# bottledspace/refraction-raytracing-dxr

Measured on AMD Instinct MI355X. Metric: Mrays/s (primary+refracted) at 1920x1080, monkey.obj, higher is better.
Workload: dtype f32

## Files before the change

refraction_raytracing_dxr_amd/csrc/rr_device.h:

```cpp
#pragma once
#include <hip/hip_runtime.h>
#include "rr_types.h"

namespace rr {

struct f3 { float x, y, z; };

__device__ __forceinline__ f3 mk3(float x, float y, float z) { f3 r; r.x = x; r.y = y; r.z = z; return r; }
__device__ __forceinline__ f3 sub3(f3 a, f3 b) { return mk3(a.x - b.x, a.y - b.y, a.z - b.z); }
__device__ __forceinline__ f3 neg3(f3 a) { return mk3(-a.x, -a.y, -a.z); }
__device__ __forceinline__ f3 scale3(f3 a, float s) { return mk3(a.x * s, a.y * s, a.z * s); }
__device__ __forceinline__ float dot3(f3 a, f3 b) { return fmaf(a.z, b.z, fmaf(a.y, b.y, a.x * b.x)); }
__device__ __forceinline__ f3 cross3(f3 a, f3 b)
{
    return mk3(fmaf(a.y, b.z, -(a.z * b.y)), fmaf(a.z, b.x, -(a.x * b.z)), fmaf(a.x, b.y, -(a.y * b.x)));
}
__device__ __forceinline__ f3 normalize3(f3 a)
{
    float inv = 1.0f / sqrtf(dot3(a, a));
    return scale3(a, inv);
}

__device__ __forceinline__ float rr_atan2f(float y, float x)
{
    const float q = fabsf(y) / fabsf(x);
    const bool big = q > 2.414213562373095f, mid = !big && q > 0.4142135623730950f;
    const float num = big ? -1.0f : mid ? q - 1.0f : q;
    const float den = big ? q : mid ? q + 1.0f : 1.0f;
    const float y0 = big ? 1.5707963267948966f : mid ? 0.7853981633974483f : 0.0f;
    const float xr = num / den;
    const float z = xr * xr;
    const float p = ((8.05374449538e-2f * z - 1.38776856032e-1f) * z + 1.99777106478e-1f) * z - 3.33329491539e-1f;
    const float r = p * z * xr + xr;
    float a = y0 + r;
    if (x < 0.0f) a = 3.14159265358979323846f - a;
    float res = y < 0.0f ? -a : a;
    if (x == 0.0f) res = y > 0.0f ? 1.5707963267948966f : -1.5707963267948966f;
    if (y == 0.0f) res = (x > 0.0f || (x == 0.0f && !__builtin_signbit(x))) ? y
                                                                             : (__builtin_signbit(y) ? -3.14159265358979323846f : 3.14159265358979323846f);
    if (x != x || y != y) res = __builtin_nanf("");
    return res;
}

__device__ __forceinline__ float rr_acosf(float x)
{
    const float ax = fabsf(x);
    const bool outer = ax > 0.5f;
    const float a = outer ? sqrtf(0.5f * (1.0f - ax)) : ax;
    const float z = a * a;
    const float p = ((((4.2163199048e-2f * z + 2.4181311049e-2f) * z + 4.5470025998e-2f) * z + 7.4953002686e-2f) * z
                     + 1.6666752422e-1f);
    const float r = p * z * a + a;
    const float two_r = 2.0f * r;
    float res = outer ? (x < 0.0f ? 3.14159265358979323846f - two_r : two_r) : 1.5707963267948966f - (x < 0.0f ? -r : r);
    if (!(x >= -1.0f && x <= 1.0f)) res = __builtin_nanf("");
    return res;
}

__device__ __forceinline__ uint32_t ftou(float f)
{
    uint32_t r;
    asm("v_cvt_u32_f32 %0, %1" : "=v"(r) : "v"(f));
    return r;
}

__device__ __forceinline__ uint32_t unorm8(float x)
{
    float c;
    asm("v_max_f32 %0, %1, 0" : "=v"(c) : "v"(x));
    asm("v_min_f32 %0, %1, 1.0" : "=v"(c) : "v"(c));
    return ftou(c * 255.0f + 0.5f);
}

struct HitRec {
    float t, U, V, ad;
    uint32_t prim;
    uint32_t leaf;
    uint32_t inst;
    bool hit;
};

struct TravCounters { uint32_t nodes, tris, node_trips = 0, leaf_trips = 0; };
__device__ __forceinline__ bool first_active_lane()
{
    return (int)(threadIdx.x & 63u) == __ffsll((long long)__ballot(1)) - 1;
}

constexpr uint32_t CULL_BACK = 0x10u, CULL_FRONT = 0x20u;
constexpr uint32_t RAY_FLAG_ACCEPT_FIRST_HIT = 0x4u;

struct BoxRay {
    f3 inv;
    f3 kn, kf;
    bool sx, sy, sz;
};
__device__ __forceinline__ void box_axis(float o, float d, float eps_w, float org, float cell, float& inv_g, float& kn, float& kf, bool& neg)
{
    const float dg = fabsf(d) < 1e-20f ? copysignf(1e-20f, d) : d;
    const float inv = __builtin_amdgcn_rcpf(dg);
    const float oi = (org - o) * inv;
    const float pad = fmaf(fabsf(oi), 1e-6f, fabsf(inv) * eps_w);
    kn = oi - pad;
    kf = oi + pad;
    inv_g = inv * cell;
    neg = inv < 0.0f;
}
__device__ __forceinline__ BoxRay box_ray(f3 O, f3 D, float scene_scale, const QGrid& g)
{
    const float eps_w = 1e-5f * fmaxf(fmaxf(fabsf(O.x), fabsf(O.y)), fmaxf(fabsf(O.z), scene_scale));
    BoxRay r;
    box_axis(O.x, D.x, eps_w, g.org[0], g.cell[0], r.inv.x, r.kn.x, r.kf.x, r.sx);
    box_axis(O.y, D.y, eps_w, g.org[1], g.cell[1], r.inv.y, r.kn.y, r.kf.y, r.sy);
    box_axis(O.z, D.z, eps_w, g.org[2], g.cell[2], r.inv.z, r.kn.z, r.kf.z, r.sz);
    return r;
}

struct NodeQ { uint4 a, b; };
__device__ __forceinline__ NodeQ load_node(const QNode* __restrict__ nodes, int node)
{
    const uint4* q = reinterpret_cast<const uint4*>(reinterpret_cast<const char*>(nodes) + (uint32_t)node);
    NodeQ n;
    n.a = q[0]; n.b = q[1];
    return n;
}
struct GlobalNodes {
    __device__ __forceinline__ NodeQ load(const QNode* __restrict__ nodes, int node) const { return load_node(nodes, node); }
};
struct LdsNodes {
    const char* base;
    __device__ __forceinline__ NodeQ load(const QNode* __restrict__, int node) const
    {
        const uint4* q = reinterpret_cast<const uint4*>(base + (uint32_t)node);
        NodeQ n;
        n.a = q[0]; n.b = q[1];
        return n;
    }
};


constexpr int TRAV_DONE = (int)0x80000000;

typedef float v2f __attribute__((ext_vector_type(2)));
__device__ __forceinline__ v2f splat2(float x) { v2f r = { x, x }; return r; }
__device__ __forceinline__ v2f mk2(float x, float y) { v2f r = { x, y }; return r; }

__device__ __forceinline__ float vmax3(float a, float b, float c) { float r; asm("v_max3_f32 %0, %1, %2, %3" : "=v"(r) : "v"(a), "v"(b), "v"(c)); return r; }
__device__ __forceinline__ float vmin3(float a, float b, float c) { float r; asm("v_min3_f32 %0, %1, %2, %3" : "=v"(r) : "v"(a), "v"(b), "v"(c)); return r; }
__device__ __forceinline__ float vmax2(float a, float b) { float r; asm("v_max_f32 %0, %1, %2" : "=v"(r) : "v"(a), "v"(b)); return r; }
__device__ __forceinline__ float vmin2(float a, float b) { float r; asm("v_min_f32 %0, %1, %2" : "=v"(r) : "v"(a), "v"(b)); return r; }

typedef _Float16 h2v __attribute__((ext_vector_type(2)));
__device__ __forceinline__ h2v as_h2(uint32_t w) { return __builtin_bit_cast(h2v, w); }
#define RR_PLANE2(word, inv, k) mk2(fmaf((float)as_h2(word).x, inv, k), fmaf((float)as_h2(word).y, inv, k))
__device__ __forceinline__ void box2_hit(const BoxRay& r, const NodeQ& n, float tmin, float tmax,
                                         bool& h0, bool& h1, float& tn0, float& tn1)
{
    const uint32_t lox = n.a.x, loy = n.a.y, loz = n.a.z, hix = n.a.w, hiy = n.b.x, hiz = n.b.y;
    const v2f nx = RR_PLANE2(r.sx ? hix : lox, r.inv.x, r.kn.x);
    const v2f ny = RR_PLANE2(r.sy ? hiy : loy, r.inv.y, r.kn.y);
    const v2f nz = RR_PLANE2(r.sz ? hiz : loz, r.inv.z, r.kn.z);
    const v2f fx = RR_PLANE2(r.sx ? lox : hix, r.inv.x, r.kf.x);
    const v2f fy = RR_PLANE2(r.sy ? loy : hiy, r.inv.y, r.kf.y);
    const v2f fz = RR_PLANE2(r.sz ? loz : hiz, r.inv.z, r.kf.z);
    tn0 = vmax2(vmax3(nx.x, ny.x, nz.x), tmin);
    tn1 = vmax2(vmax3(nx.y, ny.y, nz.y), tmin);
    const float tf0 = vmin2(vmin3(fx.x, fy.x, fz.x), tmax);
    const float tf1 = vmin2(vmin3(fx.y, fy.y, fz.y), tmax);
    h0 = tn0 <= tf0;
    h1 = tn1 <= tf1;
}

constexpr int STACK_STRIDE = 64;
template <class E> struct StackCodec;
template <> struct StackCodec<uint32_t> {
    static __device__ __forceinline__ uint32_t enc(int ref) { return (uint32_t)ref; }
    static __device__ __forceinline__ int dec(uint32_t v) { return (int)v; }
};
template <> struct StackCodec<uint16_t> {
    static __device__ __forceinline__ uint16_t enc(int ref) { const int n = ref >> 5; return (uint16_t)(n < ref ? n : ref); }
    static __device__ __forceinline__ int dec(uint16_t v) { const int s = (int)(int16_t)v, n = s << 5; return n > s ? n : s; }
};

template <class E>
__device__ __forceinline__ int node_step(const BoxRay& br, const NodeQ& n, float tmin, float tmax, E*& top, const E* floor)
{
    bool h0, h1;
    float tn0, tn1;
    box2_hit(br, n, tmin, tmax, h0, h1, tn0, tn1);
    const int c0 = (int)n.b.z, c1 = (int)n.b.w;
    const bool both = h0 && h1, swap = tn1 < tn0;
    const int nearc = (h0 && !(h1 && swap)) ? c0 : c1;
    int next = (h0 || h1) ? nearc : TRAV_DONE;
    if (both) { *top = StackCodec<E>::enc(swap ? c0 : c1); top += STACK_STRIDE; }
    if (!(h0 || h1) && top > floor) { top -= STACK_STRIDE; next = StackCodec<E>::dec(*top); }
    return next;
}

struct Diag { uint32_t* trips; uint32_t stride = 4; };
__device__ __forceinline__ void diag_trip(const Diag& d, int which = 0)
{
    if (d.trips) { const unsigned long long m = __ballot(1); if ((int)(threadIdx.x & 63u) == __ffsll((long long)m) - 1) d.trips[which * d.stride] += 1u; }
}


__device__ __forceinline__ bool tri_accept(const TriRec* __restrict__ tris, uint32_t leaf, f3 O, f3 D, float tmin, uint32_t cull,
                                           float& t, uint32_t& prim)
{
    const float4* q = reinterpret_cast<const float4*>(tris + leaf);
    float4 a = q[0], b = q[1], c = q[2];
    f3 v0 = mk3(a.x, a.y, a.z), e1 = mk3(b.x, b.y, b.z), e2 = mk3(c.x, c.y, c.z);
    prim = __float_as_uint(a.w);
    f3 pv = cross3(D, e2);
    float det = dot3(e1, pv);
    if (cull & CULL_BACK) { if (!(det > 0.0f)) return false; }
    else if (cull & CULL_FRONT) { if (!(det < 0.0f)) return false; }
    else if (!(det != 0.0f)) return false;
    f3 tv = sub3(O, v0);
    float U = dot3(tv, pv);
    f3 qv = cross3(tv, e1);
    float V = dot3(D, qv);
    float T = dot3(e2, qv);
    float ad = det;
    if (det < 0.0f) { U = -U; V = -V; T = -T; ad = -det; }
    if (U < 0.0f || V < 0.0f || U + V > ad) return false;
    t = T / ad;
    return t > tmin;
}

__device__ __forceinline__ void tri_test(const TriRec* __restrict__ tris, uint32_t leaf, f3 O, f3 D, float tmin,
                                         uint32_t cull, uint32_t inst, HitRec& best)
{
    float t;
    uint32_t prim;
    if (!tri_accept(tris, leaf, O, D, tmin, cull, t, prim)) return;
    if (t < best.t || (t == best.t && best.hit && (inst < best.inst || (inst == best.inst && prim < tris[best.leaf].prim)))) {
        best.t = t; best.leaf = leaf; best.inst = inst;
        best.hit = true;
    }
}

__device__ __forceinline__ float hit_attributes(const TriRec* __restrict__ tris, f3 O, f3 D, HitRec& best)
{
    const float4* q = reinterpret_cast<const float4*>(tris + best.leaf);
    float4 a = q[0], b = q[1], c = q[2];
    f3 v0 = mk3(a.x, a.y, a.z), e1 = mk3(b.x, b.y, b.z), e2 = mk3(c.x, c.y, c.z);
    f3 pv = cross3(D, e2);
    float det = dot3(e1, pv);
    f3 tv = sub3(O, v0);
    float U = dot3(tv, pv);
    f3 qv = cross3(tv, e1);
    float V = dot3(D, qv);
    float ad = det;
    if (det < 0.0f) { U = -U; V = -V; ad = -det; }
    best.U = U; best.V = V; best.ad = ad; best.prim = __float_as_uint(a.w);
    return det;
}

__device__ __forceinline__ void hits_begin(HitRec& best, float tmax)
{
    best.t = tmax; best.hit = false; best.prim = 0; best.leaf = 0; best.inst = 0; best.U = 0.0f; best.V = 0.0f;
    best.ad = 1.0f;
}
__device__ __forceinline__ float hit_bound(const HitRec& best) { return best.t; }
__device__ __forceinline__ bool hit_found(const HitRec& best) { return best.hit; }
__device__ __forceinline__ void leaf_test(const TriRec* __restrict__ tris, uint32_t leaf, f3 O, f3 D, float tmin, uint32_t cull,
                                          uint32_t inst, HitRec& best)
{
    tri_test(tris, leaf, O, D, tmin, cull, inst, best);
}
__device__ __forceinline__ void hits_end_blas(const TriRec* __restrict__ tris, f3 O, f3 D, HitRec& best)
{
    if (best.hit) hit_attributes(tris, O, D, best);
}

template <int KB, bool COUNT>
struct MultiHits {
    float t[KB];
    uint32_t leaf[KB], inst[KB];
    float tmax;
    uint32_t count;
};
template <int KB, bool COUNT>
__device__ __forceinline__ void hits_begin(MultiHits<KB, COUNT>& m, float tmax)
{
#pragma unroll
    for (int j = 0; j < KB; ++j) { m.t[j] = tmax; m.leaf[j] = 0; m.inst[j] = 0; }
    m.tmax = tmax; m.count = 0;
}
template <int KB, bool COUNT>
__device__ __forceinline__ float hit_bound(const MultiHits<KB, COUNT>& m) { return COUNT ? m.tmax : m.t[KB - 1]; }
template <int KB, bool COUNT>
__device__ __forceinline__ bool hit_found(const MultiHits<KB, COUNT>&) { return false; }
template <int KB, bool COUNT>
__device__ __forceinline__ void leaf_test(const TriRec* __restrict__ tris, uint32_t leaf, f3 O, f3 D, float tmin, uint32_t cull,
                                          uint32_t inst, MultiHits<KB, COUNT>& m)
{
    float t;
    uint32_t prim;
    if (!tri_accept(tris, leaf, O, D, tmin, cull, t, prim) || !(t < m.tmax)) return;
    if (COUNT) m.count++;
    bool before[KB];
#pragma unroll
    for (int j = 0; j < KB; ++j)
        before[j] = t < m.t[j] || (t == m.t[j] && (inst < m.inst[j] || (inst == m.inst[j] && prim < tris[m.leaf[j]].prim)));
    if (!before[KB - 1]) return;
#pragma unroll
    for (int j = KB - 1; j > 0; --j) {
        if (before[j - 1]) { m.t[j] = m.t[j - 1]; m.leaf[j] = m.leaf[j - 1]; m.inst[j] = m.inst[j - 1]; }
        else if (before[j]) { m.t[j] = t; m.leaf[j] = leaf; m.inst[j] = inst; }
    }
    if (before[0]) { m.t[0] = t; m.leaf[0] = leaf; m.inst[0] = inst; }
}
template <int KB, bool COUNT>
__device__ __forceinline__ void hits_end_blas(const TriRec* __restrict__, f3, f3, MultiHits<KB, COUNT>&) {}

__device__ __forceinline__ bool leaf_phase_due(int n_in)
{
    const int quarter = n_in >> 2;
    const int thr = quarter > 2 ? quarter : 2;
    return __popcll(__ballot(1)) + thr <= n_in;
}

template <bool STATS, class E, class NS = GlobalNodes, bool ANY = false, class H = HitRec>
__device__ __forceinline__ void walk_blas(const QNode* __restrict__ nodes, const TriRec* __restrict__ tris, int root, const BoxRay& br,
                                          f3 O, f3 D, float tmin, uint32_t cull, uint32_t inst, H& best, E* stk,
                                          TravCounters& cnt, const Diag dg = Diag{ nullptr }, const NS ns = NS{},
                                          bool any_lane = false)
{
    E* top = stk;
    int node = root;
    for (;;) {
        const int n_in = __popcll(__ballot(node >= 0));
        while (node >= 0) {
            if (leaf_phase_due(n_in)) break;
            diag_trip(dg);
            const NodeQ q = ns.load(nodes, node);
            if (STATS) { cnt.nodes++; if (first_active_lane()) cnt.node_trips++; }
            node = node_step(br, q, tmin, hit_bound(best), top, stk);
        }
        if (node < 0 && node != TRAV_DONE) {
            diag_trip(dg, 1);
            if (STATS) { cnt.tris++; if (first_active_lane()) cnt.leaf_trips++; }
            leaf_test(tris, (uint32_t)~node, O, D, tmin, cull, inst, best);
            if (ANY && any_lane && hit_found(best)) { top = stk; node = TRAV_DONE; }
            else if (top > stk) { top -= STACK_STRIDE; node = StackCodec<E>::dec(*top); } else node = TRAV_DONE;
        }
        if (__ballot(node != TRAV_DONE) == 0ull) break;
    }
}

template <bool STATS, class E, class NS = GlobalNodes, class H = HitRec>
__device__ __forceinline__ void trace_blas(const BlasDev& bl, f3 O, f3 D, float tmin, uint32_t cull, uint32_t inst,
                                           H& best, E* stk, TravCounters& cnt, const Diag dg = Diag{ nullptr },
                                           const NS ns = NS{})
{
    const BoxRay br = box_ray(O, D, bl.scale, bl.grid);
    walk_blas<STATS, E, NS>(bl.nodes, bl.tris, 0, br, O, D, tmin, cull, inst, best, stk, cnt, dg, ns);
    hits_end_blas(bl.tris, O, D, best);
}

template <int G> __device__ __forceinline__ uint32_t grp_next(uint32_t v);
template <int G> __device__ __forceinline__ uint32_t grp_prev(uint32_t v);
template <> __device__ __forceinline__ uint32_t grp_next<4>(uint32_t v) { return (uint32_t)__builtin_amdgcn_update_dpp(0, (int)v, 0x39, 0xf, 0xf, true); }
template <> __device__ __forceinline__ uint32_t grp_prev<4>(uint32_t v) { return (uint32_t)__builtin_amdgcn_update_dpp(0, (int)v, 0x93, 0xf, 0xf, true); }
template <> __device__ __forceinline__ uint32_t grp_next<2>(uint32_t v) { return (uint32_t)__builtin_amdgcn_update_dpp(0, (int)v, 0xb1, 0xf, 0xf, true); }
template <> __device__ __forceinline__ uint32_t grp_prev<2>(uint32_t v) { return grp_next<2>(v); }
template <int G> __device__ __forceinline__ float grp_min_f(float v)
{
    float m = fminf(v, __uint_as_float((uint32_t)__builtin_amdgcn_update_dpp(0, (int)__float_as_uint(v), 0xb1, 0xf, 0xf, true)));
    if (G == 4) m = fminf(m, __uint_as_float((uint32_t)__builtin_amdgcn_update_dpp(0, (int)__float_as_uint(m), 0x4e, 0xf, 0xf, true)));
    return m;
}
template <int G> __device__ __forceinline__ uint32_t grp_min_u(uint32_t v)
{
    uint32_t o = (uint32_t)__builtin_amdgcn_update_dpp(0, (int)v, 0xb1, 0xf, 0xf, true);
    uint32_t m = v < o ? v : o;
    if (G == 4) { o = (uint32_t)__builtin_amdgcn_update_dpp(0, (int)m, 0x4e, 0xf, 0xf, true); m = m < o ? m : o; }
    return m;
}

template <int G, bool STATS, class E>
__device__ __forceinline__ void trace_blas_group(const BlasDev& bl, bool alive, unsigned long long m_alive, f3 O, f3 D, float tmin, float tmax,
                                                 uint32_t cull, HitRec& best, E* stk, uint32_t* ww, uint32_t lane, TravCounters& cnt)
{
    const uint32_t rank = __builtin_amdgcn_mbcnt_hi((uint32_t)(m_alive >> 32), __builtin_amdgcn_mbcnt_lo((uint32_t)m_alive, 0u));
    const uint32_t n_rays = (uint32_t)__popcll(m_alive);
    if (alive) {
        ww[0 * 64 + rank] = __float_as_uint(O.x); ww[1 * 64 + rank] = __float_as_uint(O.y); ww[2 * 64 + rank] = __float_as_uint(O.z);
        ww[3 * 64 + rank] = __float_as_uint(D.x); ww[4 * 64 + rank] = __float_as_uint(D.y); ww[5 * 64 + rank] = __float_as_uint(D.z);
        ww[6 * 64 + rank] = __float_as_uint(tmax); ww[7 * 64 + rank] = cull; ww[8 * 64 + rank] = __float_as_uint(tmin);
    }
    const uint32_t g = lane / G;
    const bool work = g < n_rays;
    const uint32_t gs = work ? g : 0u;
    const f3 Og = mk3(__uint_as_float(ww[0 * 64 + gs]), __uint_as_float(ww[1 * 64 + gs]), __uint_as_float(ww[2 * 64 + gs]));
    const f3 Dg = mk3(__uint_as_float(ww[3 * 64 + gs]), __uint_as_float(ww[4 * 64 + gs]), __uint_as_float(ww[5 * 64 + gs]));
    const float tmaxg = __uint_as_float(ww[6 * 64 + gs]);
    const uint32_t cullg = ww[7 * 64 + gs];
    const float tming = __uint_as_float(ww[8 * 64 + gs]);
    asm volatile("s_waitcnt lgkmcnt(0)" ::: "memory");

    const BoxRay br = box_ray(Og, Dg, bl.scale, bl.grid);
    const QNode* __restrict__ nodes = bl.nodes;
    E* const col0 = stk - lane;
    E* top = stk;
    E* bot = stk;
    int node = (work && (lane % G) == 0u) ? 0 : TRAV_DONE;
    HitRec b;
    b.t = tmaxg; b.hit = false; b.prim = 0; b.leaf = 0; b.inst = 0; b.U = 0.0f; b.V = 0.0f; b.ad = 1.0f;
    float tq = tmaxg;
    for (;;) {
        const int n_in = __popcll(__ballot(node >= 0));
        while (node >= 0) {
            if (leaf_phase_due(n_in)) break;
            const NodeQ q = load_node(nodes, node);
            if (STATS) { cnt.nodes++; if (first_active_lane()) cnt.node_trips++; }
            node = node_step(br, q, tming, tq, top, bot);
        }
        if (node < 0 && node != TRAV_DONE) {
            if (STATS) { cnt.tris++; if (first_active_lane()) cnt.leaf_trips++; }
            tri_test(bl.tris, (uint32_t)~node, Og, Dg, tming, cullg, 0u, b);
            if (top > bot) { top -= STACK_STRIDE; node = StackCodec<E>::dec(*top); } else node = TRAV_DONE;
        }
        tq = grp_min_f<G>(b.t);
        const bool idle = node == TRAV_DONE;
        const uint32_t nb_bot = grp_next<G>((uint32_t)(bot - col0)), nb_has = grp_next<G>(top > bot ? 1u : 0u);
        const uint32_t thief_idle = grp_prev<G>(idle ? 1u : 0u);
        if (idle && nb_has) node = StackCodec<E>::dec(col0[nb_bot]);
        if (top > bot && thief_idle) bot += STACK_STRIDE;
        if (__ballot(node != TRAV_DONE) == 0ull) break;
    }
    const float tw = grp_min_f<G>(b.hit ? b.t : 3.0e38f);
    const bool cand = b.hit && b.t == tw;
    const uint32_t prim = cand ? bl.tris[b.leaf].prim : 0xffffffffu;
    const uint32_t pw = grp_min_u<G>(prim);
    const uint32_t lw = ~grp_min_u<G>((cand && prim == pw) ? ~b.leaf : 0xffffffffu);
    if (work && (lane % G) == 0u) { ww[0 * 64 + g] = __float_as_uint(tw); ww[1 * 64 + g] = tw < 3.0e38f ? lw : 0xffffffffu; }
    best.t = tmax; best.hit = false; best.prim = 0; best.leaf = 0; best.inst = 0; best.U = 0.0f; best.V = 0.0f; best.ad = 1.0f;
    if (alive) {
        const uint32_t l = ww[1 * 64 + rank];
        if (l != 0xffffffffu) { best.t = __uint_as_float(ww[0 * 64 + rank]); best.leaf = l; best.hit = true; }
    }
    asm volatile("s_waitcnt lgkmcnt(0)" ::: "memory");
    if (best.hit) hit_attributes(bl.tris, O, D, best);
}

__device__ __forceinline__ f3 xform_point(const float* m, f3 p)
{
    return mk3(((m[0] * p.x + m[1] * p.y) + m[2] * p.z) + m[3],
               ((m[4] * p.x + m[5] * p.y) + m[6] * p.z) + m[7],
               ((m[8] * p.x + m[9] * p.y) + m[10] * p.z) + m[11]);
}
__device__ __forceinline__ f3 xform_dir(const float* m, f3 p)
{
    return mk3((m[0] * p.x + m[1] * p.y) + m[2] * p.z,
               (m[4] * p.x + m[5] * p.y) + m[6] * p.z,
               (m[8] * p.x + m[9] * p.y) + m[10] * p.z);
}

__device__ __forceinline__ InstDev inst_record(const InstDev* __restrict__ insts, uint32_t ii)
{
    const uint32_t iu = (uint32_t)__builtin_amdgcn_readfirstlane((int)ii);
    InstDev r;
    if (__ballot(ii != iu) == 0ull) r = insts[iu];
    else r = insts[ii];
    return r;
}

__device__ __forceinline__ void ray_in_instance(const InstDev& in, f3 O, f3 D, f3& Oc, f3& Dc)
{
    Oc = O; Dc = D;
    if (!in.identity) { Oc = xform_point(in.inv, O); Dc = xform_dir(in.inv, D); }
}
__device__ __forceinline__ void hits_end_scene(const SceneDev& sc, f3 O, f3 D, HitRec& best)
{
    if (best.hit) {
        const InstDev in = inst_record(sc.insts, best.inst);
        f3 Oh = O, Dh = D;
        if (!in.identity) { Oh = xform_point(in.inv, O); Dh = xform_dir(in.inv, D); }
        hit_attributes(sc.pool_tris, Oh, Dh, best);
    }
}
template <int KB, bool COUNT>
__device__ __forceinline__ void hits_end_scene(const SceneDev&, f3, f3, MultiHits<KB, COUNT>&) {}

struct HitRecFace : HitRec { bool front; };
__device__ __forceinline__ void hits_end_blas(const TriRec* __restrict__ tris, f3 O, f3 D, HitRecFace& best)
{
    best.front = false;
    if (best.hit) best.front = hit_attributes(tris, O, D, best) > 0.0f;
}
__device__ __forceinline__ void hits_end_scene(const SceneDev& sc, f3 O, f3 D, HitRecFace& best)
{
    best.front = false;
    if (best.hit) {
        const InstDev in = inst_record(sc.insts, best.inst);
        f3 Oh = O, Dh = D;
        if (!in.identity) { Oh = xform_point(in.inv, O); Dh = xform_dir(in.inv, D); }
        const float det = hit_attributes(sc.pool_tris, Oh, Dh, best);
        best.front = (det > 0.0f) != ((in.flags & 0x2u) != 0u);
    }
}

template <bool STATS, bool TLAS, class E = uint32_t, class NS = GlobalNodes, bool QUERY = false, class H = HitRec>
__device__ __forceinline__ void trace_scene(const SceneDev& sc, f3 O, f3 D, float tmin, float tmax, uint32_t flags,
                                            H& best, E* stk_e, TravCounters& cnt,
                                            const Diag dg = Diag{ nullptr }, const NS ns = NS{},
                                            uint32_t ray_mask = 0xffu, bool any_lane = false)
{
    hits_begin(best, tmax);
    if (!TLAS && QUERY) {
        const BoxRay br = box_ray(O, D, sc.blas0.scale, sc.blas0.grid);
        walk_blas<STATS, E, NS, true>(sc.blas0.nodes, sc.blas0.tris, (ray_mask & 0xffu) ? 0 : TRAV_DONE, br, O, D, tmin, flags, 0u,
                                      best, stk_e, cnt, dg, ns, any_lane);
        hits_end_blas(sc.blas0.tris, O, D, best);
        return;
    }
    if (!TLAS) {
        trace_blas<STATS, E, NS>(sc.blas0, O, D, tmin, flags, 0u, best, stk_e, cnt, dg, ns);
        return;
    }
    E* stk = stk_e;
    const QNode* __restrict__ nodes = sc.pool_nodes;
    E* top = stk;
    int node = 0;
    const BoxRay br = box_ray(O, D, sc.scale, sc.grid);
    for (;;) {
        while (node >= 0) {
            const NodeQ q = load_node(nodes, node);
            if (STATS) { cnt.nodes++; if (first_active_lane()) cnt.node_trips++; }
            node = node_step(br, q, tmin, hit_bound(best), top, stk);
        }
        if (node == TRAV_DONE) break;
        if (STATS && first_active_lane()) cnt.leaf_trips++;
        const uint32_t ii = (uint32_t)~node - sc.n_pool_tris;
        const InstDev in = inst_record(sc.insts, ii);
        if (in.mask & (QUERY ? ray_mask : 0xffu)) {
            uint32_t f = flags;
            if (in.flags & 0x1u) f &= ~(CULL_BACK | CULL_FRONT);
            else if (in.flags & 0x2u) {
                if (f & CULL_BACK) f = (f & ~CULL_BACK) | CULL_FRONT;
                else if (f & CULL_FRONT) f = (f & ~CULL_FRONT) | CULL_BACK;
            }
            f3 Oc = O, Dc = D;
            if (!in.identity) { Oc = xform_point(in.inv, O); Dc = xform_dir(in.inv, D); }
            const BoxRay bi = box_ray(Oc, Dc, in.scale, in.grid);
            walk_blas<STATS, E, GlobalNodes, QUERY>(nodes, sc.pool_tris, (int)in.root, bi, Oc, Dc, tmin, f, ii, best, top, cnt,
                                                    Diag{ nullptr }, GlobalNodes{}, any_lane);
        }
        if (QUERY && any_lane && hit_found(best)) node = TRAV_DONE;
        else if (top > stk) { top -= STACK_STRIDE; node = StackCodec<E>::dec(*top); } else node = TRAV_DONE;
    }
    hits_end_scene(sc, O, D, best);
}

__device__ __forceinline__ f3 env_lookup(const SceneDev& sc, f3 r)
{
    if (!sc.env) return mk3(0.0f, 0.0f, 0.0f);
    float at = rr_atan2f(r.x, r.z);
    float ac = rr_acosf(r.y);
    float theta = (float)sc.env_w * (at / 3.14159f + 1.0f) / 2;
    float phi = (float)sc.env_h * (ac / 3.14159f);
    uint32_t ix = ftou(theta), iy = ftou(phi);
    if (ix >= (uint32_t)sc.env_w || iy >= (uint32_t)sc.env_h) return mk3(0.0f, 0.0f, 0.0f);
    float4 t = sc.env[(size_t)iy * (uint32_t)sc.env_w + ix];
    return mk3(t.x, t.y, t.z);
}

__device__ __forceinline__ f3 reflect_ray(f3 I, f3 N)
{
    float k = 2.0f * dot3(N, I);
    return mk3(I.x - k * N.x, I.y - k * N.y, I.z - k * N.z);
}

__device__ __forceinline__ bool refract_ray(f3& R, f3 I, f3 N, float eta)
{
    float c = dot3(N, I);
    float k = 1.0f - (eta * eta) * (1.0f - c * c);
    if (k < 0.0f) return false;
    float a = eta * c + sqrtf(k);
    R = normalize3(mk3(eta * I.x - a * N.x, eta * I.y - a * N.y, eta * I.z - a * N.z));
    return true;
}

__device__ __forceinline__ f3 camera_ray_dir(const float* M, float sx, float sy)
{
    f3 R;
    R.x = (sx * M[0] + sy * M[1]) + M[3];
    R.y = (sx * M[4] + sy * M[5]) + M[7];
    R.z = (sx * M[8] + sy * M[9]) + M[11];
    return normalize3(R);
}

template <bool TLAS>
__device__ __forceinline__ f3 shading_normal(const SceneDev& sc, const HitRec& h)
{
    const float4* q = reinterpret_cast<const float4*>((!TLAS ? sc.blas0.nrms : sc.pool_nrms) + h.leaf);
    float4 a = q[0], b = q[1], c = q[2];
    float u = h.U / h.ad, v = h.V / h.ad;
    f3 A = mk3(a.x, a.y, a.z);
    f3 BA = sub3(mk3(b.x, b.y, b.z), A), CA = sub3(mk3(c.x, c.y, c.z), A);
    f3 Nr = mk3(fmaf(v, CA.x, fmaf(u, BA.x, A.x)), fmaf(v, CA.y, fmaf(u, BA.y, A.y)), fmaf(v, CA.z, fmaf(u, BA.z, A.z)));
    const InstDev in = TLAS ? inst_record(sc.insts, h.inst) : InstDev{};
    if (TLAS && !in.identity) {
        const float* w = in.inv;
        Nr = mk3((w[0] * Nr.x + w[4] * Nr.y) + w[8] * Nr.z,
                 (w[1] * Nr.x + w[5] * Nr.y) + w[9] * Nr.z,
                 (w[2] * Nr.x + w[6] * Nr.y) + w[10] * Nr.z);
    }
    return normalize3(Nr);
}

__device__ __forceinline__ uint32_t wave_reduce_add(uint32_t v)
{
    uint32_t t;
    t = v + __builtin_amdgcn_update_dpp(0u, v, 0x111, 0xf, 0xf, true);
    t = t + __builtin_amdgcn_update_dpp(0u, v, 0x112, 0xf, 0xf, true);
    t = t + __builtin_amdgcn_update_dpp(0u, v, 0x113, 0xf, 0xf, true);
    t = t + __builtin_amdgcn_update_dpp(0u, t, 0x114, 0xf, 0xe, true);
    t = t + __builtin_amdgcn_update_dpp(0u, t, 0x118, 0xf, 0xc, true);
    t = t + __builtin_amdgcn_update_dpp(0u, t, 0x142, 0xa, 0xf, true);
    t = t + __builtin_amdgcn_update_dpp(0u, t, 0x143, 0xc, 0xf, true);
    return (uint32_t)__builtin_amdgcn_readlane((int)t, 63);
}

}
```

refraction_raytracing_dxr_amd/csrc/rr_render_lds.hip:

```cpp
#include <hip/hip_runtime.h>
#include "rr_render_common.h"

namespace rr {

__device__ __forceinline__ BlockPos lds_tile_block(const DispatchDev& a, const LdsDispatch& q, uint32_t u, uint32_t j)
{
    BlockPos p;
    const uint32_t tile = a.n_frames == 1u ? u : __umulhi(u, q.div_frames);
    p.frame = u - tile * a.n_frames;
    p.tile_local = tile;
    p.tile_ok = tile < a.n_local_tiles;
    p.bg = false;
    const uint32_t ty = a.tiles_x == 1u ? tile : __umulhi(tile, q.div_tiles_x), tx = tile - ty * a.tiles_x;
    p.px0 = (j & 3u) * 8u; p.py0 = (j >> 2) * 8u;
    p.x0 = tx * TILE + p.px0; p.y0 = ty * TILE + p.py0;
    return p;
}

__device__ __forceinline__ BlockPos lds_rect_block(const DispatchDev& a, const LdsDispatch& q, uint32_t u, uint32_t j)
{
    BlockPos p;
    const uint32_t strip = a.n_frames == 1u ? u : __umulhi(u, q.div_frames), per_row = q.rect_bw >> 2;
    p.frame = u - strip * a.n_frames;
    const uint32_t row = per_row == 1u ? strip : __umulhi(strip, q.div_per_row), col = strip - row * per_row;
    p.tile_local = 0u; p.tile_ok = true; p.bg = false;
    p.px0 = 0u; p.py0 = 0u;
    p.x0 = q.rx0 + col * 32u + j * 8u; p.y0 = q.ry0 + row * 8u;
    return p;
}

template <int NW, int WGS, bool STATS, bool DIAG = false>
__global__ __launch_bounds__(NW * 64, NW * WGS / 4) void k_render_lds(SceneDev sc, DispatchDev a, LdsDispatch q)
{
    typedef uint16_t E;
    __shared__ uint32_t diag_tr[3 * 16];
    __shared__ uint32_t wg_arrived;
    __shared__ unsigned long long wg_share[16];
    if (threadIdx.x == 0) wg_arrived = 0u;
    if (threadIdx.x < 16) wg_share[threadIdx.x] = 0ull;
    const unsigned long long diag_t0 = DIAG ? __builtin_amdgcn_s_memtime() : 0ull;
    unsigned long long diag_wait = 0ull, diag_render = 0ull, diag_n = 0ull;
    unsigned long long diag_worst = 0ull, diag_worst_trips = 0ull;
    if (DIAG && threadIdx.x < 48) diag_tr[threadIdx.x] = 0;
    extern __shared__ __attribute__((aligned(16))) uint32_t lds[];
    {
        const uint4* __restrict__ src = reinterpret_cast<const uint4*>(sc.blas0.nodes);
        uint4* dst = reinterpret_cast<uint4*>(lds);
        for (uint32_t i = threadIdx.x; i < q.node_bytes / 16u; i += NW * 64) dst[i] = src[i];
    }
    __syncthreads();
    const unsigned long long diag_t1 = DIAG ? __builtin_amdgcn_s_memtime() : 0ull;
    const uint32_t wave = __builtin_amdgcn_readfirstlane(threadIdx.x >> 6), lane = threadIdx.x & 63u;
    const LdsNodes ns{ reinterpret_cast<const char*>(lds) };
    MemPark park{ q.park + (size_t)(blockIdx.x * NW + wave) * ((size_t)q.park_slots * 8 * 64) + lane };
    E* stk = reinterpret_cast<E*>(reinterpret_cast<char*>(lds) + q.node_bytes) + wave * (q.stack_entries * 64u) + lane;
    const uint32_t lx = compact1by1(lane), ly = compact1by1(lane >> 1);

    LaneStats st;
    stats_clock_begin<STATS>(st);
    auto in_rect = [&](const BlockPos& bp) { return bp.x0 >= q.rx0 && bp.x0 < q.rx1 && bp.y0 >= q.ry0 && bp.y0 < q.ry1; };
    const uint32_t NQ = q.n_queues;
    uint32_t home = (blockIdx.x * NW + wave) % NQ;
    if (q.home_xcc) { uint32_t xcc; asm volatile("s_getreg_b32 %0, hwreg(HW_REG_XCC_ID)" : "=s"(xcc)); home = (xcc & 7u) % NQ; }
    uint32_t phase = 0, qi = home, tried = 0;
    for (;;) {
        BlockPos bp;
        bool have = false;
        while (!have) {
            {
                uint32_t got = 0xffffffffu, got_u = 0u;
                for (;;) {
                    const unsigned long long mine = lane < (uint32_t)NW ? wg_share[lane] : 0ull;
                    const uint32_t mh = (uint32_t)(mine >> 32);
                    const unsigned long long m = __ballot(mh != 0u && (uint32_t)mine < ((mh & 0x80000000u) ? 16u : 4u));
                    if (m == 0ull) break;
                    const unsigned long long from_own = m >> wave << wave;
                    const uint32_t sl = (uint32_t)__ffsll((long long)(from_own ? from_own : m)) - 1u;
                    unsigned long long v = 0ull;
                    if (lane == 0) v = atomicAdd(&wg_share[sl], 1ull);
                    const uint32_t lo = __builtin_amdgcn_readfirstlane((uint32_t)v), hi = __builtin_amdgcn_readfirstlane((uint32_t)(v >> 32));
                    if (hi != 0u && lo < ((hi & 0x80000000u) ? 16u : 4u)) { got = lo; got_u = hi; break; }
                }
                if (got != 0xffffffffu) {
                    if (got_u & 0x80000000u) { bp = lds_tile_block(a, q, (got_u & 0x7fffffffu) - 1u, got); have = bp.tile_ok && !in_rect(bp); }
                    else { bp = lds_rect_block(a, q, got_u - 1u, got); have = true; }
                    continue;
                }
            }
            if (phase >= 2u) break;
            const uint32_t total = phase == 0u ? q.p1_tickets : q.p2_tickets;
            uint32_t* const cnt = q.tickets + phase * LDS_QUEUES * 16u;
            bool drew = false;
            uint32_t u = 0;
            while (total != 0u && tried < NQ) {
                const uint32_t n_tickets = total > qi ? (total - qi + NQ - 1u) / NQ : 0u;
                uint32_t seen = 0u;
                if (tried != 0u) {
                    if (lane == 0) seen = __hip_atomic_load(&cnt[qi * 16u], __ATOMIC_RELAXED, __HIP_MEMORY_SCOPE_AGENT);
                    seen = __builtin_amdgcn_readfirstlane(seen);
                }
                if (seen < n_tickets) {
                    uint32_t t = 0;
                    const unsigned long long dw0 = DIAG ? __builtin_amdgcn_s_memtime() : 0ull;
                    if (lane == 0) t = atomicAdd(&cnt[qi * 16u], 1u);
                    t = __builtin_amdgcn_readfirstlane(t);
                    if (DIAG) { diag_wait += __builtin_amdgcn_s_memtime() - dw0; diag_n += 1ull; }
                    if (t < n_tickets) { u = qi + NQ * t; drew = true; break; }
                }
                ++tried;
                qi = qi + 1u == NQ ? 0u : qi + 1u;
            }
            if (!drew) { ++phase; qi = home; tried = 0u; continue; }
            if (phase == 0u) {
                if (lane == 0) wg_share[wave] = ((unsigned long long)(u + 1u) << 32) | 1ull;
                bp = lds_rect_block(a, q, u, 0u);
                have = true;
            } else {
                if (lane == 0) wg_share[wave] = ((unsigned long long)((u + 1u) | 0x80000000u) << 32) | 1ull;
                bp = lds_tile_block(a, q, u, 0u);
                have = bp.tile_ok && !in_rect(bp);
            }
        }
        if (!have) break;
        st.blocks += 1u;
        const unsigned long long dr0 = DIAG ? __builtin_amdgcn_s_memtime() : 0ull;
        const uint32_t dI0 = DIAG ? diag_tr[wave] : 0u, dL0 = DIAG ? diag_tr[16 + wave] : 0u, dS0 = DIAG ? diag_tr[32 + wave] : 0u;
        const uint32_t x = bp.x0 + lx, y = bp.y0 + ly;
        const bool may_hit = bp.x0 + 8u > a.hx0 && bp.x0 < a.hx1 && bp.y0 + 8u > a.hy0 && bp.y0 < a.hy1;
        if (STATS && !may_hit) st.bg_blocks += 1u;
        if (x < a.W && y < a.H) {
            const CamDev& cb = a.cams[bp.frame];
            st.pixels += 1;
            const f3 acc = render_pixel<STATS, false, DIAG, E, LdsNodes>(sc, a, cb, x, y, may_hit, stk, ns, park, st, Diag{ DIAG ? &diag_tr[wave] : nullptr, 16 });
            const size_t o = a.compact_out == 0u ? (size_t)y * a.W + x
                                                : (size_t)bp.tile_local * (TILE * TILE) + (bp.py0 + ly) * TILE + (bp.px0 + lx);
            store_pixel(a, a.out_rgba8 + (size_t)bp.frame * a.frame_stride,
                        a.out_f32 ? a.out_f32 + (size_t)bp.frame * a.frame_stride : nullptr, o, acc);
        }
        if (DIAG) {
            const unsigned long long dt = __builtin_amdgcn_s_memtime() - dr0;
            diag_render += dt; diag_n += 1ull << 32;
            if (dt > diag_worst) {
                diag_worst = dt;
                diag_worst_trips = (unsigned long long)(diag_tr[wave] - dI0) | ((unsigned long long)(diag_tr[16 + wave] - dL0) << 20) |
                                   ((unsigned long long)(diag_tr[32 + wave] - dS0) << 40);
            }
        }
    }
    if (DIAG && lane == 0) {
        unsigned long long* d = a.diag + (size_t)(blockIdx.x * NW + wave) * 8;
        d[0] = diag_wait; d[1] = diag_render; d[2] = diag_n; d[3] = __builtin_amdgcn_s_memtime() - diag_t0;
        d[4] = diag_worst; d[5] = diag_worst_trips; d[6] = diag_t1 - diag_t0; d[7] = diag_tr[wave] | ((unsigned long long)diag_tr[16 + wave] << 32);
    }
    flush_stats<STATS>(a, st, blockIdx.x * NW + wave, lane);
    if (lane == 0) {
        const uint32_t w_arrived = atomicAdd(&wg_arrived, 1u);
        if (w_arrived + 1u == (uint32_t)NW) {
            const uint32_t arrived = atomicAdd(&q.tickets[2u * LDS_QUEUES * 16u], 1u);
            if (arrived + 1u == gridDim.x) {
                for (uint32_t k = 0; k <= 2u * LDS_QUEUES; ++k) atomicExch(&q.tickets[k * 16u], 0u);
            }
        }
    }
}

constexpr struct { int nw, wgs; } LDS_SHAPES[] = { { 12, 2 }, { 16, 2 }, { 16, 1 } };
static size_t lds_shape_bytes(int i, uint32_t node_bytes, uint32_t stack_entries) { return (size_t)node_bytes + (size_t)LDS_SHAPES[i].nw * stack_entries * 64 * sizeof(uint16_t); }

int lds_kernel_shape(uint32_t node_bytes, uint32_t stack_entries, size_t* lds_bytes, int min_shape)
{
    for (int i = min_shape < 0 ? 0 : min_shape; i < 3; ++i) {
        const size_t need = lds_shape_bytes(i, node_bytes, stack_entries);
        if (need <= (size_t)(160 * 1024) / LDS_SHAPES[i].wgs - 512) { if (lds_bytes) *lds_bytes = need; return i; }
        if (min_shape <= 0) break;
    }
    return -1;
}

template <int SHAPE, bool STATS, bool DIAG = false>
static hipError_t launch_lds_nw(const SceneDev& sc, const DispatchDev& a, const LdsDispatch& q, int n_cus, hipStream_t s)
{
    constexpr int NW = LDS_SHAPES[SHAPE].nw, WGS = LDS_SHAPES[SHAPE].wgs;
    static const hipError_t attr = hipFuncSetAttribute(reinterpret_cast<const void*>(&k_render_lds<NW, WGS, STATS, DIAG>), hipFuncAttributeMaxDynamicSharedMemorySize, 159 * 1024);
    if (attr != hipSuccess) return attr;
    if (!DIAG) set_render_kernel_name("k_render_lds<%d, %d, %s, false>", NW, WGS, STATS ? "true" : "false");
    hipLaunchKernelGGL((k_render_lds<NW, WGS, STATS, DIAG>), dim3((uint32_t)n_cus * WGS), dim3(NW * 64), lds_shape_bytes(SHAPE, q.node_bytes, q.stack_entries), s, sc, a, q);
    return hipGetLastError();
}

hipError_t launch_render_lds(const SceneDev& sc, const DispatchDev& a, LdsDispatch q, int n_cus, bool stats, hipStream_t s, int min_shape)
{
    if (a.n_blocks == 0) return hipSuccess;
    const int shape = lds_kernel_shape(q.node_bytes, q.stack_entries, nullptr, min_shape);
    if (shape < 0) return hipErrorInvalidValue;
    {
        const uint32_t grid = (uint32_t)n_cus * (uint32_t)LDS_SHAPES[shape].wgs;
        if (q.n_queues > grid) q.n_queues = grid;
        if (q.n_queues > LDS_QUEUES) q.n_queues = LDS_QUEUES;
        if (q.n_queues < 1u) q.n_queues = 1u;
    }
    q.p2_tickets = a.n_local_tiles * a.n_frames;
    if (q.rx1 > q.rx0 && q.ry1 > q.ry0) {
        q.rx0 &= ~31u;
        q.rx1 = (q.rx1 + 31u) & ~31u;
    }
    const bool rect = q.rx1 > q.rx0 && q.ry1 > q.ry0;
    q.rect_bw = rect ? (q.rx1 - q.rx0) / 8u : 0u;
    q.p1_tickets = !rect ? 0u : (q.rect_bw / 4u) * ((q.ry1 - q.ry0) / 8u) * a.n_frames;
    if ((uint64_t)q.p2_tickets * a.n_frames >= 0xffffffffull || (uint64_t)q.p1_tickets * a.n_frames >= 0xffffffffull) return hipErrorInvalidValue;
    q.div_frames = (uint32_t)(0x100000000ull / a.n_frames) + 1u;
    q.div_tiles_x = (uint32_t)(0x100000000ull / a.tiles_x) + 1u;
    q.div_per_row = rect ? (uint32_t)(0x100000000ull / (q.rect_bw / 4u)) + 1u : 0u;
    static_assert(sizeof LDS_SHAPES / sizeof LDS_SHAPES[0] == 3, "lds_kernel_shape and the rungs below");
    if (a.diag) return launch_lds_nw<0, false, true>(sc, a, q, n_cus, s);
    if (shape == 0) return stats ? launch_lds_nw<0, true>(sc, a, q, n_cus, s) : launch_lds_nw<0, false>(sc, a, q, n_cus, s);
    if (shape == 1) return stats ? launch_lds_nw<1, true>(sc, a, q, n_cus, s) : launch_lds_nw<1, false>(sc, a, q, n_cus, s);
    return stats ? launch_lds_nw<2, true>(sc, a, q, n_cus, s) : launch_lds_nw<2, false>(sc, a, q, n_cus, s);
}

}
```

Baseline: 31330.

## Add LDS kernel variant with absolute LDS child addresses and int16 stack refs

Adds a k_render_lds_d16 variant that rewrites child node offsets to absolute LDS addresses while copying nodes into shared memory. Node loads then use address_space(3) pointers directly with no base add, and the traversal stack stores raw int16 refs with no encode/decode shifts. The push is skipped when no lane in the wave needs it. Statics are placed inside the dynamic LDS region, and the variant is only used when the BVH is at most 32KB, shape 0 fits, and there are at least 24 frames. This brings extra code paths and a ballot per node step.

Measured after the change: 30770. -1.8%, worse.

```diff
diff --git a/refraction_raytracing_dxr_amd/csrc/rr_device.h b/refraction_raytracing_dxr_amd/csrc/rr_device.h
--- a/refraction_raytracing_dxr_amd/csrc/rr_device.h
+++ b/refraction_raytracing_dxr_amd/csrc/rr_device.h
@@ -125,6 +125,7 @@
 }
 struct GlobalNodes {
     __device__ __forceinline__ NodeQ load(const QNode* __restrict__ nodes, int node) const { return load_node(nodes, node); }
+    __device__ __forceinline__ int root() const { return 0; }
 };
 struct LdsNodes {
     const char* base;
@@ -135,6 +136,20 @@
         n.a = q[0]; n.b = q[1];
         return n;
     }
+    __device__ __forceinline__ int root() const { return 0; }
+};
+struct LdsDirectNodes {
+    uint32_t base;
+    __device__ __forceinline__ NodeQ load(const QNode* __restrict__, int node) const
+    {
+        typedef uint32_t u32x4 __attribute__((ext_vector_type(4)));
+        const __attribute__((address_space(3))) u32x4* q = (const __attribute__((address_space(3))) u32x4*)(uintptr_t)(uint32_t)node;
+        const u32x4 a = q[0], b = q[1];
+        NodeQ n;
+        n.a = make_uint4(a.x, a.y, a.z, a.w); n.b = make_uint4(b.x, b.y, b.z, b.w);
+        return n;
+    }
+    __device__ __forceinline__ int root() const { return (int)base; }
 };
 
 
@@ -173,12 +188,20 @@
 constexpr int STACK_STRIDE = 64;
 template <class E> struct StackCodec;
 template <> struct StackCodec<uint32_t> {
+    static constexpr bool SKIP_EMPTY_PUSH = false;
     static __device__ __forceinline__ uint32_t enc(int ref) { return (uint32_t)ref; }
     static __device__ __forceinline__ int dec(uint32_t v) { return (int)v; }
 };
 template <> struct StackCodec<uint16_t> {
+    static constexpr bool SKIP_EMPTY_PUSH = false;
     static __device__ __forceinline__ uint16_t enc(int ref) { const int n = ref >> 5; return (uint16_t)(n < ref ? n : ref); }
     static __device__ __forceinline__ int dec(uint16_t v) { const int s = (int)(int16_t)v, n = s << 5; return n > s ? n : s; }
+};
+struct Ref16 { int16_t v; };
+template <> struct StackCodec<Ref16> {
+    static constexpr bool SKIP_EMPTY_PUSH = true;
+    static __device__ __forceinline__ Ref16 enc(int ref) { return Ref16{ (int16_t)ref }; }
+    static __device__ __forceinline__ int dec(Ref16 e) { return (int)e.v; }
 };
 
 template <class E>
@@ -191,7 +214,10 @@
     const bool both = h0 && h1, swap = tn1 < tn0;
     const int nearc = (h0 && !(h1 && swap)) ? c0 : c1;
     int next = (h0 || h1) ? nearc : TRAV_DONE;
-    if (both) { *top = StackCodec<E>::enc(swap ? c0 : c1); top += STACK_STRIDE; }
+    if (!StackCodec<E>::SKIP_EMPTY_PUSH || __ballot(both) != 0ull) {
+        if (StackCodec<E>::SKIP_EMPTY_PUSH) asm volatile("");
+        if (both) { *top = StackCodec<E>::enc(swap ? c0 : c1); top += STACK_STRIDE; }
+    }
     if (!(h0 || h1) && top > floor) { top -= STACK_STRIDE; next = StackCodec<E>::dec(*top); }
     return next;
 }
@@ -355,7 +381,7 @@
                                            const NS ns = NS{})
 {
     const BoxRay br = box_ray(O, D, bl.scale, bl.grid);
-    walk_blas<STATS, E, NS>(bl.nodes, bl.tris, 0, br, O, D, tmin, cull, inst, best, stk, cnt, dg, ns);
+    walk_blas<STATS, E, NS>(bl.nodes, bl.tris, ns.root(), br, O, D, tmin, cull, inst, best, stk, cnt, dg, ns);
     hits_end_blas(bl.tris, O, D, best);
 }
 
diff --git a/refraction_raytracing_dxr_amd/csrc/rr_render_lds.hip b/refraction_raytracing_dxr_amd/csrc/rr_render_lds.hip
--- a/refraction_raytracing_dxr_amd/csrc/rr_render_lds.hip
+++ b/refraction_raytracing_dxr_amd/csrc/rr_render_lds.hip
@@ -1,4 +1,5 @@
 #include <hip/hip_runtime.h>
+#include <type_traits>
 #include "rr_render_common.h"
 
 namespace rr {
@@ -29,29 +30,41 @@
     return p;
 }
 
-template <int NW, int WGS, bool STATS, bool DIAG = false>
-__global__ __launch_bounds__(NW * 64, NW * WGS / 4) void k_render_lds(SceneDev sc, DispatchDev a, LdsDispatch q)
-{
-    typedef uint16_t E;
-    __shared__ uint32_t diag_tr[3 * 16];
-    __shared__ uint32_t wg_arrived;
-    __shared__ unsigned long long wg_share[16];
+constexpr uint32_t LDS_D16_BYTES = 160u * 1024u / 2u - 512u;
+constexpr uint32_t LDS_D16_STATICS = LDS_D16_BYTES - 256u;
+constexpr uint32_t LDS_D16_NODE_BYTES = 32768u;
+static_assert(LDS_D16_NODE_BYTES / sizeof(QNode) + 1u <= 32768u, "a mesh on the direct-ref kernel has at most one leaf more than nodes: ~leaf must fit a signed half");
+
+template <int NW, int WGS, bool STATS, bool DIAG, bool D16>
+__device__ __forceinline__ void render_lds(const SceneDev& sc, const DispatchDev& a, const LdsDispatch& q, uint32_t* lds,
+                                           uint32_t& wg_arrived, unsigned long long* wg_share, uint32_t* diag_tr)
+{
+    typedef typename std::conditional<D16, Ref16, uint16_t>::type E;
+    typedef typename std::conditional<D16, LdsDirectNodes, LdsNodes>::type NS;
     if (threadIdx.x == 0) wg_arrived = 0u;
     if (threadIdx.x < 16) wg_share[threadIdx.x] = 0ull;
     const unsigned long long diag_t0 = DIAG ? __builtin_amdgcn_s_memtime() : 0ull;
     unsigned long long diag_wait = 0ull, diag_render = 0ull, diag_n = 0ull;
     unsigned long long diag_worst = 0ull, diag_worst_trips = 0ull;
     if (DIAG && threadIdx.x < 48) diag_tr[threadIdx.x] = 0;
-    extern __shared__ __attribute__((aligned(16))) uint32_t lds[];
+    const uint32_t lds_base = (uint32_t)reinterpret_cast<uintptr_t>(lds);
     {
         const uint4* __restrict__ src = reinterpret_cast<const uint4*>(sc.blas0.nodes);
         uint4* dst = reinterpret_cast<uint4*>(lds);
-        for (uint32_t i = threadIdx.x; i < q.node_bytes / 16u; i += NW * 64) dst[i] = src[i];
+        for (uint32_t i = threadIdx.x; i < q.node_bytes / 16u; i += NW * 64) {
+            uint4 v = src[i];
+            if (D16 && (i & 1u)) {
+                if ((int)v.z >= 0) v.z += lds_base;
+                if ((int)v.w >= 0) v.w += lds_base;
+            }
+            dst[i] = v;
+        }
     }
     __syncthreads();
     const unsigned long long diag_t1 = DIAG ? __builtin_amdgcn_s_memtime() : 0ull;
     const uint32_t wave = __builtin_amdgcn_readfirstlane(threadIdx.x >> 6), lane = threadIdx.x & 63u;
-    const LdsNodes ns{ reinterpret_cast<const char*>(lds) };
+    NS ns;
+    if constexpr (D16) ns.base = lds_base; else ns.base = reinterpret_cast<const char*>(lds);
     MemPark park{ q.park + (size_t)(blockIdx.x * NW + wave) * ((size_t)q.park_slots * 8 * 64) + lane };
     E* stk = reinterpret_cast<E*>(reinterpret_cast<char*>(lds) + q.node_bytes) + wave * (q.stack_entries * 64u) + lane;
     const uint32_t lx = compact1by1(lane), ly = compact1by1(lane >> 1);
@@ -131,7 +144,7 @@
         if (x < a.W && y < a.H) {
             const CamDev& cb = a.cams[bp.frame];
             st.pixels += 1;
-            const f3 acc = render_pixel<STATS, false, DIAG, E, LdsNodes>(sc, a, cb, x, y, may_hit, stk, ns, park, st, Diag{ DIAG ? &diag_tr[wave] : nullptr, 16 });
+            const f3 acc = render_pixel<STATS, false, DIAG, E, NS>(sc, a, cb, x, y, may_hit, stk, ns, park, st, Diag{ DIAG ? &diag_tr[wave] : nullptr, 16 });
             const size_t o = a.compact_out == 0u ? (size_t)y * a.W + x
                                                 : (size_t)bp.tile_local * (TILE * TILE) + (bp.py0 + ly) * TILE + (bp.px0 + lx);
             store_pixel(a, a.out_rgba8 + (size_t)bp.frame * a.frame_stride,
@@ -164,6 +177,25 @@
     }
 }
 
+template <int NW, int WGS, bool STATS, bool DIAG = false>
+__global__ __launch_bounds__(NW * 64, NW * WGS / 4) void k_render_lds(SceneDev sc, DispatchDev a, LdsDispatch q)
+{
+    __shared__ uint32_t diag_tr[3 * 16];
+    __shared__ uint32_t wg_arrived;
+    __shared__ unsigned long long wg_share[16];
+    extern __shared__ __attribute__((aligned(16))) uint32_t lds[];
+    render_lds<NW, WGS, STATS, DIAG, false>(sc, a, q, lds, wg_arrived, wg_share, diag_tr);
+}
+
+template <int NW, int WGS, bool STATS>
+__global__ __launch_bounds__(NW * 64, NW * WGS / 4) void k_render_lds_d16(SceneDev sc, DispatchDev a, LdsDispatch q)
+{
+    extern __shared__ __attribute__((aligned(32))) uint32_t lds[];
+    char* const statics = reinterpret_cast<char*>(lds) + LDS_D16_STATICS;
+    render_lds<NW, WGS, STATS, false, true>(sc, a, q, lds, *reinterpret_cast<uint32_t*>(statics + 128),
+                                            reinterpret_cast<unsigned long long*>(statics), nullptr);
+}
+
 constexpr struct { int nw, wgs; } LDS_SHAPES[] = { { 12, 2 }, { 16, 2 }, { 16, 1 } };
 static size_t lds_shape_bytes(int i, uint32_t node_bytes, uint32_t stack_entries) { return (size_t)node_bytes + (size_t)LDS_SHAPES[i].nw * stack_entries * 64 * sizeof(uint16_t); }
 
@@ -185,6 +217,29 @@
     if (attr != hipSuccess) return attr;
     if (!DIAG) set_render_kernel_name("k_render_lds<%d, %d, %s, false>", NW, WGS, STATS ? "true" : "false");
     hipLaunchKernelGGL((k_render_lds<NW, WGS, STATS, DIAG>), dim3((uint32_t)n_cus * WGS), dim3(NW * 64), lds_shape_bytes(SHAPE, q.node_bytes, q.stack_entries), s, sc, a, q);
+    return hipGetLastError();
+}
+
+constexpr uint32_t LDS_D16_MIN_FRAMES = 24;
+static bool lds_d16_fits(uint32_t node_bytes, uint32_t stack_entries, uint32_t n_frames)
+{
+    return n_frames >= LDS_D16_MIN_FRAMES && node_bytes <= LDS_D16_NODE_BYTES && lds_shape_bytes(0, node_bytes, stack_entries) <= LDS_D16_STATICS;
+}
+
+template <bool STATS>
+static hipError_t launch_lds_d16(const SceneDev& sc, const DispatchDev& a, const LdsDispatch& q, int n_cus, hipStream_t s)
+{
+    constexpr int NW = LDS_SHAPES[0].nw, WGS = LDS_SHAPES[0].wgs;
+    static const hipError_t attr = [] {
+        const void* const f = reinterpret_cast<const void*>(&k_render_lds_d16<NW, WGS, STATS>);
+        hipFuncAttributes fa;
+        hipError_t e = hipFuncGetAttributes(&fa, f);
+        if (e == hipSuccess && fa.sharedSizeBytes != 0) e = hipErrorInvalidDeviceFunction;
+        return e != hipSuccess ? e : hipFuncSetAttribute(f, hipFuncAttributeMaxDynamicSharedMemorySize, 159 * 1024);
+    }();
+    if (attr != hipSuccess) return attr;
+    set_render_kernel_name("k_render_lds_d16<%d, %d, %s>", NW, WGS, STATS ? "true" : "false");
+    hipLaunchKernelGGL((k_render_lds_d16<NW, WGS, STATS>), dim3((uint32_t)n_cus * WGS), dim3(NW * 64), LDS_D16_BYTES, s, sc, a, q);
     return hipGetLastError();
 }
 
@@ -213,6 +268,7 @@
     q.div_per_row = rect ? (uint32_t)(0x100000000ull / (q.rect_bw / 4u)) + 1u : 0u;
     static_assert(sizeof LDS_SHAPES / sizeof LDS_SHAPES[0] == 3, "lds_kernel_shape and the rungs below");
     if (a.diag) return launch_lds_nw<0, false, true>(sc, a, q, n_cus, s);
+    if (shape == 0 && lds_d16_fits(q.node_bytes, q.stack_entries, a.n_frames)) return stats ? launch_lds_d16<true>(sc, a, q, n_cus, s) : launch_lds_d16<false>(sc, a, q, n_cus, s);
     if (shape == 0) return stats ? launch_lds_nw<0, true>(sc, a, q, n_cus, s) : launch_lds_nw<0, false>(sc, a, q, n_cus, s);
     if (shape == 1) return stats ? launch_lds_nw<1, true>(sc, a, q, n_cus, s) : launch_lds_nw<1, false>(sc, a, q, n_cus, s);
     return stats ? launch_lds_nw<2, true>(sc, a, q, n_cus, s) : launch_lds_nw<2, false>(sc, a, q, n_cus, s);
```
